# SamsungLabs/Metis

Hardware: NVIDIA H100
Metric: candidate plans evaluated/sec (higher is better)
Workload: dtype f64

## Files before the change

metis_b200/csrc/metis_eval.cuh:

```cuda
#pragma once

#include <stdint.h>
#include <string.h>
#include <math.h>

#include "../../include/metis_b200.h"

#if defined(__CUDACC__)
#define MB_HD __host__ __device__ __forceinline__
#define MB_HD_NOINLINE __host__ __device__ __noinline__
#else
#define MB_HD inline
#define MB_HD_NOINLINE inline
#endif

namespace metis {

constexpr int kH = 7;
constexpr double kMemCoef = 5.0;
constexpr uint8_t kDropped = 0xFF;

struct Tables {
    MetisProblem p;
    const int16_t *key_index;
// ... 45 lines not shown
    if (i < d.dpk) return (double)(i - d.ratio) / (double)p.num_layers;
    const double bw = bw_first[0] * 1048576.0;
    if (i < d.pp_hidden) {
        const int dp = 1 << (i - d.dpk);
        return (double)(2 * (dp - 1)) / ((double)dp * bw);
    }
    if (i < d.pp_vocab) return (double)((int64_t)(i - d.pp_hidden) * p.sequence_length * p.hidden_size) / bw;
    if (i >= d.dsub) return norm_lc[(i - d.dsub) / kH] / 7.0;
    if (i >= d.psub) {
        const int j = i - d.psub, r = j / kH;
        double acc = 0.0;
        for (int t = 0; t < r; ++t) acc += norm_lc[t];
        return r < p.norm_len ? acc + norm_lc[r] * ((double)(j - r * kH) / 7.0) : acc;
    }
    const int e = i - d.pp_vocab;
    const int mbs = e / p.num_tp, tpc = e - mbs * p.num_tp;
    return ((double)((int64_t)mbs * p.sequence_length * p.vocab_size) / (double)(1 << tpc)) / bw;
}

MB_HD void bind_derived(Tables &T, const double *base) {
    const DerivedLayout d = derived_layout(T.p);
    T.dlay = base + d.dlay;
    T.inv_exec = base + d.inv_exec;
    T.ratio = base + d.ratio;
    T.dpk = base + d.dpk;
    T.pp_hidden = base + d.pp_hidden;
    T.pp_vocab = base + d.pp_vocab;
    T.psub = base + d.psub;
    T.dsub = base + d.dsub;
}

struct PlanDesc {
    uint32_t ordinal;
    int ns;
    int S;
    int label;
    int batches;
    const uint8_t *row;
    uint64_t geo;
};

MB_HD uint64_t pack_geo(int64_t row_offset, int S, int label, int ns, int div) {
    return (uint64_t)(row_offset & 0xFFFFFFFFLL) | ((uint64_t)((S - 1) & 0xFF) << 32) | ((uint64_t)((label - 1) & 0xFF) << 40) |
           ((uint64_t)(ns & 0xFF) << 48) | ((uint64_t)(div & 0xFF) << 56);
}

enum BalancerPath {
    kPathVerifyFailed = 0,
    kPathSeqForward = 1,
    kPathIrregular = 2,
    kPathMiddle = 3,
    kPathFirstGe = 4,
    kPathTail = 5,
};

struct Serial {
    static constexpr bool kUniform = false;
    MB_HD void mark(int) const {}
    MB_HD void note(int) const {}
    MB_HD void converge() const {}
    MB_HD void rejoin(bool) {}
};
#if defined(__CUDACC__)
struct Lockstep : Serial {
    unsigned mask;
    __device__ Lockstep() : mask(0xFFFFFFFFu) {}
    __device__ void converge() const { __syncwarp(mask); }
    __device__ void rejoin(bool p) { mask = __ballot_sync(0xFFFFFFFFu, p); }
};
#endif
struct SerialUniform : Serial {
    static constexpr bool kUniform = true;
};

constexpr uint64_t kOnes = 0x0101010101010101ULL;

constexpr uint16_t kBroke = 0x8000;
constexpr uint16_t kTaken = 0x4000;
constexpr uint16_t kPos = 0x3FFF;

template <int MAXS, int MAXL>
struct Scratch {
    double perf[MAXS];
    double capa[MAXS];
    double mstate[MAXS];
    double extra[MAXS];
    uint16_t fe[MAXS];
    uint16_t first[MAXS], lastl[MAXS], cnt[MAXS];
    uint16_t part[MAXS + 1];
    uint16_t rs[MAXS + 1];
    uint8_t gcode[MAXS];
    uint8_t tpc[MAXS];
    uint8_t lstk[MAXS];
    uint8_t got[MAXS];
    uint64_t ownerw[MAXL / 8 + 1];
    uint64_t subw[MAXL];
    static_assert(MAXL >= MAXS, "after the vote, subw holds one double per stage (adjust_performance, get_cost)");
};

MB_HD double py_sum_range(const double *x, int a, int b) {
    if (a >= b) return 0.0;
    double f = 0.0 + x[a];
    double c = 0.0;
    for (int i = a + 1; i < b; ++i) {
        const double v = x[i];
        const double t = f + v;
        if (fabs(f) >= fabs(v)) c += (f - t) + v;
        else c += (v - t) + f;
        f = t;
    }
    if (c != 0.0 && isfinite(c)) f += c;
    return f;
}

MB_HD_NOINLINE double py_sum_range_compact(const double *x, int a, int b) {
    if (a >= b) return 0.0;
    double f = 0.0 + x[a];
    double c = 0.0;
#pragma unroll 1
    for (int i = a + 1; i < b; ++i) {
        const double v = x[i];
        const double t = f + v;
        if (fabs(f) >= fabs(v)) c += (f - t) + v;
        else c += (v - t) + f;
        f = t;
    }
    if (c != 0.0 && isfinite(c)) f += c;
    return f;
}

template <class X>
MB_HD double sum_range(const double *x, int a, int b) {
    if constexpr (X::kUniform) return py_sum_range_compact(x, a, b);
    else return py_sum_range(x, a, b);
}

MB_HD void fill_range_sums(const double *row, int L, int a, double *out) {
    const int n = L + 1;
    double f = 0.0 + row[a];
    double c = 0.0;
    out[(size_t)(a + 1) * n + a] = f;
#if defined(__CUDA_ARCH__)
#pragma unroll 1
#endif
    for (int i = a + 1; i < L; ++i) {
        const double v = row[i];
        const double t = f + v;
        if (fabs(f) >= fabs(v)) c += (f - t) + v;
        else c += (v - t) + f;
        f = t;
// ... 38 lines not shown
        ++n;
    }
    MB_HD double result() const {
        double r = f;
        if (c != 0.0 && isfinite(c)) r += c;
        return r;
    }
};

MB_HD double pow2_neg(int k) {
    const uint64_t bits = (uint64_t)(1023 - k) << 52;
    double d;
    memcpy(&d, &bits, sizeof(d));
    return d;
}

MB_HD int type_of_rank(const Tables &T, int ns, int rank) {
    const int nt = T.p.num_types;
    const int32_t *end = T.run_end + ns * nt;
    const uint8_t *typ = T.run_type + ns * nt;
#pragma unroll 1
    for (int k = 0; k < nt; ++k)
        if (rank < end[k]) return typ[k];
    return typ[nt - 1];
}

MB_HD int type_of_q10(const Tables &T, int ns, int idx) {
    const int nt = T.p.num_types;
    const int32_t *end = T.q10_end + ns * nt;
    const uint8_t *typ = T.run_type + ns * nt;
#pragma unroll 1
    for (int k = 0; k < nt; ++k)
        if (idx < end[k]) return typ[k];
    return typ[nt - 1];
}

MB_HD int key_of(const Tables &T, int type, int tpc, int bs) {
    if (tpc >= T.p.num_tp || bs < 1 || bs > T.p.num_bs) return -1;
    return T.key_index[(type * T.p.num_tp + tpc) * T.p.num_bs + (bs - 1)];
}

template <int MAXS, int MAXL>
MB_HD int fwd_start(const Scratch<MAXS, MAXL> &w, int s) {
    if (s == 0) return 0;
    const uint16_t e = w.fe[s - 1];
    return (e & kPos) + ((e & kBroke) ? 1 : 0);
}

template <int MAXS, int MAXL>
MB_HD bool fwd_nonempty(const Scratch<MAXS, MAXL> &w, int s) {
    return (int)(w.fe[s] & kPos) > fwd_start(w, s);
}

MB_HD void sub_store(uint64_t *subw, int j, int stage) {
    reinterpret_cast<uint8_t *>(subw)[(j / kH) * 8 + (j % kH)] = (uint8_t)stage;
}

MB_HD int popc64(uint64_t v) {
#if defined(__CUDA_ARCH__)
    return __popcll(v);
#else
    return __builtin_popcountll(v);
#endif
}
MB_HD int ctz64(uint64_t v) {
#if defined(__CUDA_ARCH__)
    return __ffsll((long long)v) - 1;
#else
    return __builtin_ctzll(v);
#endif
}
MB_HD int popc32(uint32_t v) {
#if defined(__CUDA_ARCH__)
    return __popc(v);
#else
    return __builtin_popcount(v);
#endif
}
MB_HD int ctz32(uint32_t v) {
#if defined(__CUDA_ARCH__)
    return __ffs((int)v) - 1;
#else
    return __builtin_ctz(v);
#endif
}
MB_HD int clz32(uint32_t v) {
#if defined(__CUDA_ARCH__)
    return __clz((int)v);
#else
    return __builtin_clz(v);
#endif
}
MB_HD int clz64(uint64_t v) {
#if defined(__CUDA_ARCH__)
    return __clzll((long long)v);
#else
    return __builtin_clzll(v);
#endif
}

MB_HD uint64_t swar_eq(uint64_t x, int c) {
    const uint64_t y = x ^ ((uint64_t)c * kOnes);
    const uint64_t lo7 = 0x7F7F7F7F7F7F7F7FULL;
    return ~((((y & lo7) + lo7) | y) | lo7);
}

MB_HD int swar_count(uint64_t x, int c) { return popc64(swar_eq(x, c) & 0x0080808080808080ULL); }

MB_HD int layer_owner(uint64_t v, bool plurality) {
    if (plurality) {
        int best = 0, own = (int)kDropped;
#pragma unroll 1
        for (int q = 0; q < kH; ++q) {
            const int cq = (int)((v >> (8 * q)) & 0xFF);
            const int n = swar_count(v, cq);
            if (n > best || (n == best && cq < own)) { best = n; own = cq; }
        }
        return own;
    }
    const int c3 = (int)((v >> 24) & 0xFF);
    if (swar_count(v, c3) * 2 > kH) return c3;
    const int c0 = (int)(v & 0xFF), c1 = (int)((v >> 8) & 0xFF), c2 = (int)((v >> 16) & 0xFF);
    if (swar_count(v, c0) * 2 > kH) return c0;
    if (c1 != c0 && swar_count(v, c1) * 2 > kH) return c1;
    if (c2 != c1 && c2 != c0 && swar_count(v, c2) * 2 > kH) return c2;
    return (int)kDropped;
}

template <int MAXS, int MAXL, class X>
MB_HD int balance_run(const Tables &T, int S, Scratch<MAXS, MAXL> &w, const X &x) {
    const int L = T.p.num_layers;
    if (T.p.norm_len < L) return METIS_FATAL_INDEX;
    const double *dlay = T.dlay;
    const double *lc = T.norm_lc;
    const int N = kH * L;
    const int lim = (N - 1 - kH) > 0 ? (N - 1 - kH) : 0;
    const int last = S - 1;
    int broken = METIS_FATAL_NONE;

#pragma unroll (X::kUniform ? 1 : 0)
    for (int s = 0; s < S; ++s) { w.capa[s] = w.perf[s]; w.got[s] = 0; w.cnt[s] = 0; }

    x.mark(10);
    int k = 0, sTop = -1;
    bool topSkip = false;
    if (S > 1) {
        int s = 0, j = 0;
        double c = w.capa[0];
#pragma unroll (X::kUniform ? 1 : 0)
        for (int r = 0; r + 1 < L; ++r) {
            const double d = dlay[r];
            const int nsub = (r == L - 2) ? kH - 1 : kH;
            const int s_in = s;
            uint64_t v = 0;
#pragma unroll
            for (int q = 0; q < kH; ++q) {
                if (q < nsub) {
                    if (s < last) {
                        if (c > d) {
                            c -= d;
                            v |= (uint64_t)(uint32_t)s << (8 * q);
                        } else {
                            w.capa[s] = c;
                            w.fe[s] = (uint16_t)(j | kBroke);
                            ++s;
                            c = w.capa[s];
                        }
                    }
                    ++j;
                }
            }
            if (s_in < last) w.subw[r] = v;
        }
        if (s < last) {
            x.note(kPathTail);
            w.capa[s] = c;
            w.fe[s] = (uint16_t)lim;
#pragma unroll (X::kUniform ? 1 : 0)
            for (int t = s + 1; t < last; ++t) w.fe[t] = (uint16_t)lim;
            k = lim;
            sTop = s;
        } else {
            k = (w.fe[last - 1] & kPos) + 1;
            sTop = last - 1;
            topSkip = true;
        }
    }

    x.mark(11);
    x.converge();
    int m;
    {
        double c = w.capa[last];
        const double dl = dlay[L - 1];
#pragma unroll (X::kUniform ? 1 : 0)
        for (int i = 0; i < kH; ++i) c -= dl;
        m = N - kH;
        int sp = S - 2;
#pragma unroll (X::kUniform ? 1 : 0)
        while (m > 0) {
            const int j = m - 1;
            bool un = (j >= k);
            if (!un) {
#pragma unroll (X::kUniform ? 1 : 0)
                while (sp >= 0 && (!(w.fe[sp] & kBroke) || (int)(w.fe[sp] & kPos) > j)) --sp;
                un = (sp >= 0 && (int)(w.fe[sp] & kPos) == j);
            }
            if (!un) break;
            const double d = dlay[j / kH];
            if (!(c > d)) break;
            c -= d;
            m = j;
            if (j < k) w.fe[sp] |= kTaken;
        }
        w.capa[last] = c;
    }

    x.mark(12);
    x.converge();
    {
        int start = 0;
#pragma unroll (X::kUniform ? 1 : 0)
        for (int s = 0; s < last; ++s) {
            const uint16_t e = w.fe[s];
            const int pos = e & kPos;
            const int next_start = pos + ((e & kBroke) ? 1 : 0);
            if ((e & (kBroke | kTaken)) != kBroke) { start = next_start; continue; }
            const int j = pos;
            int lo = 0;
            if (pos > start) {
                lo = s;
            } else {
                x.note(kPathIrregular);
#pragma unroll (X::kUniform ? 1 : 0)
                for (int u = s;; --u) {
                    if (u < s) {
                        const int t = w.lstk[u];
                        const bool above = (t == last) || (fwd_nonempty(w, t) && fwd_start(w, t) > j);
                        if (!above) { lo = t; break; }
                    }
                    if (fwd_nonempty(w, u)) { lo = u; break; }
                    if (u == 0) break;
                }
            }
            int hi = s + 1;
            if (hi < last && !((int)(w.fe[hi] & kPos) > next_start && !w.got[hi])) {
                ++hi;
#pragma unroll (X::kUniform ? 1 : 0)
                while (hi < last && (!fwd_nonempty(w, hi) || w.got[hi])) ++hi;
            }
            if (lo > hi) { broken = METIS_FATAL_SCRATCH; hi = lo; }
            int pick = lo;
            double best = w.capa[lo];
#pragma unroll (X::kUniform ? 1 : 0)
            for (int t = lo + 1; t <= hi; ++t)
                if (w.capa[t] > best) { best = w.capa[t]; pick = t; }
            w.capa[pick] -= dlay[j / kH];
            w.lstk[s] = (uint8_t)pick;
            w.got[pick] = 1;
            sub_store(w.subw, j, pick);
            start = next_start;
        }
    }
    x.converge();
    const int nblk = m - k;
    if (nblk > 0) x.note(kPathMiddle);
    {
        int below = -1;
#pragma unroll (X::kUniform ? 1 : 0)
        for (int t = 0; t < nblk; ++t) {
            const int j = k + t;
            int lo = 0;
            if (below >= 0) lo = below;
            else if (sTop >= 0) {
#pragma unroll (X::kUniform ? 1 : 0)
                for (int u = sTop;; --u) {
                    if (u < sTop || topSkip) {
                        const uint16_t eu = w.fe[u];
                        if ((eu & (kBroke | kTaken)) == kBroke) {
                            const int t2 = w.lstk[u];
                            if (t2 != last) { lo = t2; break; }
                        }
                    }
                    if (fwd_nonempty(w, u)) { lo = u; break; }
                    if (u == 0) break;
                }
            }
            int pick = lo;
            double best = w.capa[lo];
#pragma unroll (X::kUniform ? 1 : 0)
            for (int t2 = lo + 1; t2 <= last; ++t2)
                if (w.capa[t2] > best) { best = w.capa[t2]; pick = t2; }
            w.capa[pick] -= dlay[j / kH];
            if (pick != last) below = pick;
            sub_store(w.subw, j, pick);
        }
    }

    x.mark(13);
    x.converge();
    int run_own = (int)kDropped, run_first = 0, run_len = 0;
#pragma unroll (X::kUniform ? 1 : 0)
    for (int r = 0; r < L; ++r) {
        const int nlow = m - kH * r;
        int own;
        if (nlow <= 0) {
            own = last;
        } else {
            uint64_t v = w.subw[r];
            if (nlow < kH) {
                const uint64_t mask = (1ULL << (8 * nlow)) - 1ULL;
                v = (v & mask) | (((uint64_t)last * kOnes) & ~mask);
            }
            v |= 0xFF00000000000000ULL;
            own = layer_owner(v, (T.p.corrected & METIS_FIX_Q5) != 0);
        }
        reinterpret_cast<uint8_t *>(w.ownerw)[r] = (uint8_t)own;
        {
            if (own == run_own) ++run_len;
            else {
                if (run_own != (int)kDropped) {
                    if (w.cnt[run_own] == 0) w.first[run_own] = (uint16_t)run_first;
                    w.lastl[run_own] = (uint16_t)(r - 1);
                    w.cnt[run_own] = (uint16_t)(w.cnt[run_own] + run_len);
                }
                run_own = own; run_first = r; run_len = 1;
            }
        }
    }
    if (run_own != (int)kDropped) {
        if (w.cnt[run_own] == 0) w.first[run_own] = (uint16_t)run_first;
        w.lastl[run_own] = (uint16_t)(L - 1);
        w.cnt[run_own] = (uint16_t)(w.cnt[run_own] + run_len);
    }
    x.mark(14);
    x.converge();
    uint8_t *owner = reinterpret_cast<uint8_t *>(w.ownerw);
#pragma unroll (X::kUniform ? 1 : 0)
    for (int s = 0; s < S; ++s)
        w.capa[s] = w.cnt[s] ? w.perf[s] - range_sum<X>(T, kRangeNorm, 0, lc, w.first[s], (int)w.lastl[s] + 1) : w.perf[s];

    x.mark(15);
    x.converge();
#pragma unroll (X::kUniform ? 1 : 0)
    for (int n = 1; n <= 3; ++n) {
        int top = 0x7FFFFFFF;
        double maxc = -INFINITY;
#pragma unroll (X::kUniform ? 1 : 0)
        for (int t = 0; t < S; ++t)
            if (w.capa[t] > maxc) { maxc = w.capa[t]; top = t; }
        if (top == 0x7FFFFFFF) top = 0;
        int nb = -1;
        double val = INFINITY;
        if (top - 1 >= 0 && w.capa[top - 1] < val) { nb = top - 1; val = w.capa[top - 1]; }
        if (top + 1 < S && w.capa[top + 1] < val) { nb = top + 1; }
        if (nb < 0 || w.cnt[nb] <= 1) break;
        const int layer = (top > nb) ? w.lastl[nb] : w.first[nb];
        const double dl = lc[layer];
        const double ntop = w.capa[top] - dl;
        const double nnb = w.capa[nb] + dl;
        double newmax = -INFINITY;
#pragma unroll (X::kUniform ? 1 : 0)
        for (int t = 0; t < S; ++t) {
            const double v = (t == top) ? ntop : (t == nb) ? nnb : w.capa[t];
            if (v > newmax) newmax = v;
        }
        if (newmax > maxc) break;
        owner[layer] = (uint8_t)top;
        w.capa[top] = ntop;
        w.capa[nb] = nnb;
        if (top > nb) { int r = layer - 1; while (owner[r] != nb) --r; w.lastl[nb] = (uint16_t)r; }
        else          { int r = layer + 1; while (owner[r] != nb) ++r; w.first[nb] = (uint16_t)r; }
        if (w.cnt[top] == 0) { w.first[top] = (uint16_t)layer; w.lastl[top] = (uint16_t)layer; }
        else {
            if (layer < (int)w.first[top]) w.first[top] = (uint16_t)layer;
            if (layer > (int)w.lastl[top]) w.lastl[top] = (uint16_t)layer;
        }
        ++w.cnt[top];
        --w.cnt[nb];
    }

    x.mark(16);
    x.converge();
    w.part[0] = 0;
#pragma unroll (X::kUniform ? 1 : 0)
    for (int s = 0; s < S; ++s) w.part[s + 1] = (uint16_t)(w.part[s] + w.cnt[s]);
    return broken;
}

struct HSplit {
    int nruns;
    int type[METIS_MAX_TYPES];
    int n[METIS_MAX_TYPES];
    int base[METIS_MAX_TYPES];
    int plus[METIS_MAX_TYPES];
};

MB_HD_NOINLINE int partition_data(const Tables &T, int ns, int rank_lo, int count, int dp, int tpc, int bs,
                                  HSplit &out, uint32_t &aux, bool q10 = false) {
    const int gsz = count / dp;
    double perf[METIS_MAX_TYPES];
    PySum total;
    out.nruns = 0;
#pragma unroll 1
    for (int i = 0; i < dp; ++i) {
        const int t = q10 ? type_of_q10(T, ns, rank_lo + i * gsz) : type_of_rank(T, ns, rank_lo + i * gsz);
        if (out.nruns == 0 || out.type[out.nruns - 1] != t) {
            const int key = key_of(T, t, tpc, 1);
            if (key < 0) { aux = ((uint32_t)tpc << 16) | 1u; return METIS_FATAL_KEY_EXEC; }
            const double e = T.exec_full[key];
            if (e == 0.0) return METIS_FATAL_ZERODIV;
            out.type[out.nruns] = t;
            out.n[out.nruns] = 0;
            perf[out.nruns] = 1. / e;
            ++out.nruns;
        }
        ++out.n[out.nruns - 1];
        total.add(perf[out.nruns - 1]);
    }
    const double tot = total.result();
    double frac[METIS_MAX_TYPES];
    int assigned = 0;
#pragma unroll 1
    for (int r = 0; r < out.nruns; ++r) {
        const double v = (double)bs * (perf[r] / tot);
        const int b = (int)v;
        out.base[r] = b;
        out.plus[r] = 0;
        frac[r] = v - (double)b;
        assigned += b * out.n[r];
    }
    int rem = bs - assigned;
// ... 232 lines not shown
    MB_HD bool stage_time(int s, double &len) {
        const bool one_type = ONE || T.p.num_types == 1;
        const int g = w.gcode[s], tpc = w.tpc[s];
        const int a = one_type ? 0 : rank_start(s), b = a + (1 << g);
        const int la = w.part[s], lb = w.part[s + 1];
        const int ldp = g - tpc;
        const int ta = one_type ? 0 : type_of_rank(T, pd.ns, a);
        const int tb = one_type ? 0 : type_of_rank(T, pd.ns, b - 1);
        len = 0.0;
        if (ta != tb) return hetero_exec_cost(a, b, 1 << ldp, tpc, la, lb, len) != 0;
        const int key = key_of(T, ta, tpc, bs_total >> ldp);
        if (key < 0) return true;
        len = range_sum<X>(T, kRangeLc, key, T.lc + (size_t)key * T.p.lpad, la, lb);
        return false;
    }

    MB_HD void stage_terms(int s, int nstage, double &pp, double &dpc, double &upd) const {
        const int per = T.p.devices_per_node;
        const int Lm = T.p.num_layers;
        const bool ubw = T.p.uniform_bw != 0;
        const int g = w.gcode[s], tpc = w.tpc[s];
        const int la = w.part[s], lb = w.part[s + 1];
        const int ldp = g - tpc;
        const int mbs = bs_total >> ldp;
        const double inv_tp = pow2_neg(tpc);
        pp = 0.0;
        if (s < nstage - 1) {
            if (ubw) {
                pp = (lb == Lm - 1) ? T.pp_vocab[mbs * T.p.num_tp + tpc] : T.pp_hidden[mbs];
            } else {
                double act;
                if (lb == Lm - 1)
                    act = (double)((int64_t)mbs * T.p.sequence_length * T.p.vocab_size) * inv_tp;
                else
                    act = (double)((int64_t)mbs * T.p.sequence_length * T.p.hidden_size);
                pp = act / (bw_of_node_range(rank_start(s) / per, (rank_start(s + 2) - 1) / per) * 1048576.0);
            }
        }
        int ntr = lb - la;
        double params = 0.0;
        if (la == 0) { params += T.p.input_params * inv_tp; --ntr; }
        if (lb == Lm) { params += T.p.output_params * inv_tp; --ntr; }
        params += T.p.transformer_params * inv_tp * (double)ntr;
        if (ubw) dpc = T.dpk[ldp] * params;
        else {
            const int dp = 1 << ldp;
            dpc = (double)(2 * (dp - 1)) / ((double)dp * (dp_bandwidth(rank_start(s), dp, 1 << tpc) * 1048576.0)) * params;
        }
        upd = T.p.optimizer_time * inv_tp * T.ratio[lb - la];
    }


    MB_HD int compute_performance() {
#pragma unroll (X::kUniform ? 1 : 0)
        for (int s = 0; s < pd.S; ++s) {
            double p;
            const int rc = stage_performance(s, p);
            w.perf[s] = p;
            w.extra[s] = encode_error(rc, aux);
        }
        x.converge();
        PySum total;
#pragma unroll (X::kUniform ? 1 : 0)
        for (int s = 0; s < pd.S; ++s) {
            if (w.extra[s] != 0.0) return decode_error(w.extra[s], aux);
            total.add(w.perf[s]);
        }
        const double tot = total.result();
        if (tot == 0.0) return METIS_FATAL_ZERODIV;
#pragma unroll (X::kUniform ? 1 : 0)
        for (int s = 0; s < pd.S; ++s) w.perf[s] = w.perf[s] / tot;
        return 0;
    }

    MB_HD_NOINLINE int hetero_memory_demand(int s, int type0, double &demand) {
        const int la = w.part[s], lb = w.part[s + 1], tpc = w.tpc[s];
        HSplit hs;
        const int rc = partition_data(T, pd.ns, 0, T.p.q10_devices, dp_of(s), tpc, bs_total, hs, aux, true);
        if (rc) return rc;
#pragma unroll (X::kUniform ? 1 : 0)
        for (int r = 0; r < hs.nruns; ++r)
#pragma unroll (X::kUniform ? 1 : 0)
            for (int i = 0; i < hs.n[r]; ++i) {
                const int h = hs.base[r] + (i < hs.plus[r] ? 1 : 0);
#pragma unroll (X::kUniform ? 1 : 0)
                for (int bit = 30; bit >= 0; --bit) {
                    const int piece = 1 << bit;
                    if (!(h & piece)) continue;
                    const int key = key_of(T, type0, tpc, piece);
                    if (key < 0) { aux = ((uint32_t)tpc << 16) | (uint32_t)piece; return METIS_FATAL_KEY_MEMORY; }
                    demand += range_sum<X>(T, kRangeMem, key, T.mem + (size_t)key * T.p.lpad, la, lb) * kMemCoef;
                }
            }
        return 0;
    }

    MB_HD_NOINLINE int memory_demand_own_type(int s, double &demand) {
        const int la = w.part[s], lb = w.part[s + 1], tpc = w.tpc[s], g = w.gcode[s];
        const int a = rank_start(s), b = a + (1 << g);
        const int ta = type_of_rank(T, pd.ns, a), tb = type_of_rank(T, pd.ns, b - 1);
        if (ta == tb) {
            const int bs = bs_total >> (g - tpc);
            const int key = key_of(T, ta, tpc, bs);
            if (key < 0) { aux = ((uint32_t)tpc << 16) | (uint32_t)bs; return METIS_FATAL_KEY_MEMORY; }
            demand += range_sum<SerialUniform>(T, kRangeMem, key, T.mem + (size_t)key * T.p.lpad, la, lb) * kMemCoef;
            return 0;
        }
        HSplit hs;
        const int rc = partition_data(T, pd.ns, a, b - a, 1 << (g - tpc), tpc, bs_total, hs, aux);
        if (rc) return rc;
        double worst = 0.0;
#pragma unroll 1
        for (int r = 0; r < hs.nruns; ++r)
#pragma unroll 1
            for (int v = 0; v < 2; ++v) {
                const int cntv = v ? hs.plus[r] : hs.n[r] - hs.plus[r];
                const int h = hs.base[r] + v;
                if (cntv <= 0 || h == 0) continue;
                double need = 0.0;
#pragma unroll 1
                for (int bit = 30; bit >= 0; --bit) {
                    const int piece = 1 << bit;
                    if (!(h & piece)) continue;
                    const int key = key_of(T, hs.type[r], tpc, piece);
                    if (key < 0) { aux = ((uint32_t)tpc << 16) | (uint32_t)piece; return METIS_FATAL_KEY_MEMORY; }
                    need += range_sum<SerialUniform>(T, kRangeMem, key, T.mem + (size_t)key * T.p.lpad, la, lb) * kMemCoef;
                }
                if (need > worst) worst = need;
            }
        demand += worst;
        return 0;
    }

    MB_HD_NOINLINE int adjust_performance() {
        const int S = pd.S;
        double *ratio = reinterpret_cast<double *>(w.subw);
        double need = 0.;
        PySum avail_sum;
#pragma unroll (X::kUniform ? 1 : 0)
        for (int s = 0; s < S; ++s) {
            double av, adj, extra;
            stage_adjust(s, av, adj, extra);
            w.capa[s] = av;
            w.mstate[s] = adj;
            need += extra;
            avail_sum.add(av);
        }
        if (avail_sum.result() < need) return 1;
#pragma unroll (X::kUniform ? 1 : 0)
        for (int s = 0; s < S; ++s) w.extra[s] = 0.;
        int guard = 0;
#pragma unroll (X::kUniform ? 1 : 0)
        while (need > 0.01) {
            PySum tot;
#pragma unroll (X::kUniform ? 1 : 0)
            for (int s = 0; s < S; ++s) tot.add(w.capa[s] > 0.001 ? w.perf[s] : 0.0);
            const double tmp_total = tot.result();
#pragma unroll (X::kUniform ? 1 : 0)
            for (int s = 0; s < S; ++s)
                ratio[s] = w.capa[s] > 0.001 ? w.perf[s] / tmp_total : 0.0;
#pragma unroll (X::kUniform ? 1 : 0)
            for (int s = 0; s < S; ++s) {
                const double av = w.capa[s];
                const double want = need * ratio[s];
                const double give = want > av ? av : want;
                w.extra[s] += give;
                w.capa[s] -= give;
                need -= give;
            }
            if (++guard > 4096) return -METIS_FATAL_HANG;
        }
#pragma unroll (X::kUniform ? 1 : 0)
        for (int s = 0; s < S; ++s) w.perf[s] = w.extra[s] + w.mstate[s];
        return 0;
    }

    MB_HD int memory_phase(int attempt) {
        const int S = pd.S;
#pragma unroll (X::kUniform ? 1 : 0)
        for (int s = 0; s < S; ++s) {
            double md, state;
            const int rc = stage_memory(s, md, state);
            w.extra[s] = md;
            w.capa[s] = state;
            w.mstate[s] = encode_error(rc, aux);
            if (tap) { tap->demand[s] = md; tap->state[s] = state; }
        }
        x.converge();
        bool oom = false;
#pragma unroll (X::kUniform ? 1 : 0)
        for (int s = 0; s < S; ++s) {
            if (w.mstate[s] != 0.0) return -decode_error(w.mstate[s], aux);
            if (w.capa[s] < 0) oom = true;
        }
        if (!oom) {
#pragma unroll (X::kUniform ? 1 : 0)
            for (int s = 0; s < S; ++s) w.mstate[s] = w.capa[s];
            return 1;
        }
        if (attempt >= 3) return 0;
        x.mark(21);
        const int rc = adjust_performance();
        if (rc < 0) return rc;
        return rc == 1 ? 0 : 2;
    }

    template <class Sink>
    MB_HD_NOINLINE int partition_layer(Sink &sink) {
#pragma unroll (X::kUniform ? 1 : 0)
        for (int attempt = 1; attempt <= 3; ++attempt) {
            sink.balancer_run();
            const int rc = balance_run<MAXS, MAXL>(T, pd.S, w, x);
            if (rc) return -rc;
            const int r = memory_phase(attempt);
            if (r == 1) return attempt;
            if (r <= 0) return r;
        }
        return 0;
    }

    MB_HD double bw_of_node_range(int n0, int n1) const {
        const int per = T.p.devices_per_node;
        if (n0 == n1) return T.bw_first[type_of_q10(T, pd.ns, n0 * per)];
        double slow = INFINITY;
        const int nt = T.p.num_types;
        const int32_t *end = T.q10_end + pd.ns * nt;
        const uint8_t *typ = T.run_type + pd.ns * nt;
        int lo = 0;
#pragma unroll (X::kUniform ? 1 : 0)
        for (int k = 0; k < nt; ++k) {
            const int hi = end[k];
            if (hi > lo && n0 * per < hi && (n1 + 1) * per > lo) {
                const double v = T.bw_min[typ[k]];
                if (v < slow) slow = v;
            }
            lo = hi;
        }
        return slow;
    }

    MB_HD double dp_bandwidth(int a, int dp, int tp) const {
        const int per = T.p.devices_per_node;
        double slow = INFINITY;
#pragma unroll (X::kUniform ? 1 : 0)
        for (int d = 0; d < dp; ++d) {
            const int n0 = (a + d) / per;
            int nlast = n0;
            bool multi = false;
            double gmin = INFINITY;
            int tprev = -1;
#pragma unroll (X::kUniform ? 1 : 0)
            for (int i = 0; i < tp; ++i) {
                const int node = (a + d + i * dp) / per;
                if (node != nlast) { multi = true; nlast = node; }
                const int t = type_of_q10(T, pd.ns, node * per);
                if (t != tprev) { const double v = T.bw_min[t]; if (v < gmin) gmin = v; tprev = t; }
            }
// ... 7 lines not shown
        HSplit hs;
        uint32_t dummy;
        if (partition_data(T, pd.ns, a, b - a, dp, tpc, bs_total, hs, dummy)) return 1;
        len = -INFINITY;
#pragma unroll (X::kUniform ? 1 : 0)
        for (int r = 0; r < hs.nruns; ++r)
#pragma unroll (X::kUniform ? 1 : 0)
            for (int v = 0; v < 2; ++v) {
                const int cntv = v ? hs.plus[r] : hs.n[r] - hs.plus[r];
                const int h = hs.base[r] + v;
                if (cntv <= 0 || h == 0) continue;
                double acc = 0.;
#pragma unroll (X::kUniform ? 1 : 0)
                for (int bit = 30; bit >= 0; --bit) {
                    const int piece = 1 << bit;
                    if (!(h & piece)) continue;
                    if (piece > T.p.max_bs) return 1;
                    const int key = key_of(T, hs.type[r], tpc, piece);
                    if (key < 0) return 1;
                    acc += range_sum<X>(T, kRangeLc, key, T.lc + (size_t)key * T.p.lpad, la, lb);
                }
                if (acc > len) len = acc;
            }
        return 0;
    }

    MB_HD int fb_sync_cost(int a, int b, int tpc, int mbs, double &out) const {
        const int nt = T.p.num_types;
        const int32_t *end = T.run_end + pd.ns * nt;
        const uint8_t *typ = T.run_type + pd.ns * nt;
        double mx = -INFINITY;
        int lo = 0;
#pragma unroll (X::kUniform ? 1 : 0)
        for (int k = 0; k < nt; ++k) {
            const int hi = end[k];
            if ((a > lo ? a : lo) < (b < hi ? b : hi)) {
                const int key = key_of(T, typ[k], tpc, mbs);
                if (key < 0) return 1;
                const double v = T.fb_sync[key];
                if (v == 0.0) return 1;
                if (v > mx) mx = v;
            }
            lo = hi;
        }
        out = mx;
        return 0;
    }

    MB_HD int get_cost(double &cost_out) {
        const bool one_type = ONE || T.p.num_types == 1;
        const int nstage = pd.label < pd.S ? pd.label : pd.S;
        if (T.p.q10_devices < T.p.total_devices && rank_start(nstage) > T.p.q10_devices) return 1;
        bool bad = false;
#pragma unroll (X::kUniform ? 1 : 0)
        for (int s = 0; s < nstage; ++s) {
            double len;
            if (stage_time(s, len)) bad = true;
            w.capa[s] = len;
        }
        if (bad) return 1;
        double *ppterm = reinterpret_cast<double *>(w.subw);
        double max_len = -INFINITY, max_upd = -INFINITY, max_dp = -INFINITY;
#pragma unroll (X::kUniform ? 1 : 0)
        for (int s = 0; s < nstage; ++s) {
            double dpc, upd;
            stage_terms(s, nstage, ppterm[s], dpc, upd);
            if (w.capa[s] > max_len) max_len = w.capa[s];
            if (dpc > max_dp) max_dp = dpc;
            if (upd > max_upd) max_upd = upd;
        }
        PySum lens_sum;
        double pp_cost = 0., fb_sync = 0.;
#pragma unroll (X::kUniform ? 1 : 0)
        for (int s = 0; s < nstage; ++s) {
            lens_sum.add(w.capa[s]);
            if (s < nstage - 1) pp_cost += ppterm[s];
        }
        {
            const int s = nstage - 1;
            const int a = one_type ? 0 : rank_start(s), b = a + group(s);
            double v;
            if (fb_sync_cost(a, b, w.tpc[s], bs_total >> (w.gcode[s] - w.tpc[s]), v)) return 1;
            fb_sync = v * (double)pd.batches;
        }
        const double exec = ((double)(pd.batches - 1) * max_len) + lens_sum.result();
        const double bg = T.p.batch_generator * (double)pd.batches;
        cost_out = exec + fb_sync + max_upd + max_dp + pp_cost + bg;
        if (tap) { tap->cost[0] = exec; tap->cost[1] = fb_sync; tap->cost[2] = max_upd; tap->cost[3] = max_dp; tap->cost[4] = pp_cost; }
        return 0;
    }

    template <class Sink>
    MB_HD_NOINLINE void run(const PlanDesc &plan, Sink &sink, int only_step = -1) {
        const int ok = begin(plan);
        if (ok < 0) { sink.fatal(plan.ordinal, METIS_FATAL_SCRATCH, 0); return; }
        if (ok == 0) return;
        bool started = false, have_state = false;
        int nrep = 0, step = 0;
#pragma unroll (X::kUniform ? 1 : 0)
        for (;;) {
            if (nrep == 1) return;
            int attempt = 0;
#pragma unroll (X::kUniform ? 1 : 0)
            for (;;) {
                if (!started) started = true;
                else if (!next_strategy(have_state)) return;
                if (!valid()) continue;
                sink.partition_call();
                int rc = compute_performance();
                if (rc) { sink.fatal(pd.ordinal, rc, aux); return; }
                attempt = partition_layer(sink);
                if (attempt < 0) { sink.fatal(pd.ordinal, -attempt, aux); return; }
                have_state = attempt > 0;
                if (attempt > 0) break;
            }
            nrep = attempt;
            double cost;
            if (get_cost(cost) == 0) sink.emit(pd, step, nrep, cost, w.tpc, w.part);
            else sink.keyerror();
            if (only_step >= 0 && step == only_step) return;
            ++step;
        }
    }
};

template <int MAXS, int MAXL, bool ONE, class X = Serial, class Sink>
MB_HD bool first_task(const Tables &T, Scratch<MAXS, MAXL> &w, Sink &sink, bool has, const PlanDesc &plan, int &chain_hint,
                      int &resume) {
    PlanEvaluator<MAXS, MAXL, X, ONE> ev(T, w);
// ... 116 lines not shown
```

metis_b200/csrc/metis_search.cu:

```cuda
#include <cuda_runtime.h>
#include <cooperative_groups.h>
#include <stdint.h>
#include <stdio.h>
#include <stdlib.h>
#include <string.h>

#include "metis_eval.cuh"
#include "metis_coop.cuh"
#include "metis_warp.cuh"
#include "metis_trace.cuh"
#include "metis_rows.cuh"

namespace cg = cooperative_groups;

namespace metis {

#ifndef METIS_THREADS
#define METIS_THREADS 256
#endif
#ifndef METIS_MIN_BLOCKS
#define METIS_MIN_BLOCKS 3
#endif
#ifndef METIS_MIN_BLOCKS_BIG
#define METIS_MIN_BLOCKS_BIG METIS_MIN_BLOCKS
// ... 171 lines not shown
    } else {
        lo = find_block(sp, ordinal);
    }
    const MetisPlanBlock b = sp.blocks[lo];
    const int64_t rel = ordinal - b.first_ordinal;
    const int64_t row = rel / sp.num_div;
    const int div = (int)(rel - row * sp.num_div);
    pd.ordinal = (uint32_t)ordinal;
    pd.ns = b.ns_idx;
    pd.S = b.num_stage;
    pd.label = b.label_stage;
    pd.batches = __ldg(&sp.batches[div]);
    const int64_t off = b.rows_offset + row * b.num_stage;
    pd.row = sp.rows + off;
    pd.geo = pack_geo(off, b.num_stage, b.label_stage, b.ns_idx, div);
    return true;
}

__device__ __forceinline__ void decode_task(const MetisPlanSpace &sp, uint64_t hdr, uint64_t geo, PlanDesc &pd) {
    pd.ordinal = (uint32_t)hdr;
    pd.geo = geo;
    pd.row = sp.rows + (geo & 0xFFFFFFFFULL);
    pd.S = (int)((geo >> 32) & 0xFF) + 1;
    pd.label = (int)((geo >> 40) & 0xFF) + 1;
    pd.ns = (int)((geo >> 48) & 0xFF);
    pd.batches = __ldg(&sp.batches[(geo >> 56) & 0xFF]);
}

__device__ __forceinline__ bool rec_less(double c0, uint32_t o0, uint32_t s0, double c1, uint32_t o1, uint32_t s1) {
    if (c0 < c1) return true;
    if (c0 > c1) return false;
    if (o0 != o1) return o0 < o1;
    return s0 < s1;
}

struct DeviceOut {
    MetisRecord *records;
    long long capacity;
    uint8_t *detail;
    int detail_stride;
    unsigned long long *counters;
    MetisRecord *block_best;
};

struct DeviceSink {
    const DeviceOut &o;
    unsigned int n_part, n_run, n_key;
    double best_cost;
    uint32_t best_ord, best_step, best_meta;
    bool leader;
    __device__ DeviceSink(const DeviceOut &out)
        : o(out), n_part(0), n_run(0), n_key(0), best_cost(INFINITY), best_ord(0xFFFFFFFFu), best_step(0xFFFFu),
          best_meta(0), leader(true) {}
    __device__ void phase(int) {}
    __device__ void partition_call() { n_part += leader ? 1u : 0u; }
    __device__ void balancer_run() { n_run += leader ? 1u : 0u; }
    __device__ void keyerror() { n_key += leader ? 1u : 0u; }
    __device__ void fatal(uint32_t ordinal, int code, uint32_t aux) {
        if (!leader) return;
        const unsigned long long key = ((unsigned long long)ordinal << 32) | ((unsigned long long)(code & 0xFF) << 24) |
                                       (unsigned long long)(((aux >> 16) & 0xFF) << 16) | (aux & 0xFFFF);
        atomicMin(&o.counters[4], key);
    }
    __device__ void emit(const PlanDesc &pd, int step, int nrep, double cost, const uint8_t *tpc, const uint16_t *part) {
        if (!leader) return;
        const unsigned long long slot = atomicAdd(&o.counters[0], 1ULL);
        if ((long long)slot < o.capacity) {
            MetisRecord r;
            r.cost = cost; r.ordinal = pd.ordinal; r.step = (uint16_t)step;
            r.num_repartition = (uint8_t)nrep; r.num_stage = (uint8_t)pd.S;
            o.records[slot] = r;
            if (o.detail) {
                uint8_t *d = o.detail + (size_t)slot * o.detail_stride;
                for (int s = 0; s < pd.S; ++s) { d[s] = (uint8_t)(pd.row[s] - tpc[s]); d[pd.S + s] = tpc[s]; }
                for (int s = 0; s <= pd.S; ++s) d[2 * pd.S + s] = (uint8_t)part[s];
            }
        }
        if (rec_less(cost, pd.ordinal, (uint32_t)step, best_cost, best_ord, best_step)) {
            best_cost = cost; best_ord = pd.ordinal; best_step = (uint32_t)step;
            best_meta = ((uint32_t)nrep << 8) | (uint32_t)pd.S;
        }
    }
};

__device__ __forceinline__ void finish_block(const DeviceSink &sink, const DeviceOut &out, int slot) {
    __shared__ double s_cost[32];
    __shared__ uint32_t s_ord[32], s_step[32], s_meta[32];
    const unsigned full = 0xFFFFFFFFu;
    const unsigned np = __reduce_add_sync(full, sink.n_part);
    const unsigned nr = __reduce_add_sync(full, sink.n_run);
    const unsigned nk = __reduce_add_sync(full, sink.n_key);
    const int lane = threadIdx.x & 31, warp = threadIdx.x >> 5;
    if (lane == 0) {
        if (np) atomicAdd(&out.counters[1], (unsigned long long)np);
        if (nr) atomicAdd(&out.counters[2], (unsigned long long)nr);
        if (nk) atomicAdd(&out.counters[3], (unsigned long long)nk);
    }
    double c = sink.best_cost;
    uint32_t o = sink.best_ord, st = sink.best_step, mt = sink.best_meta;
    for (int d = 16; d > 0; d >>= 1) {
        const double c2 = __shfl_xor_sync(full, c, d);
        const uint32_t o2 = __shfl_xor_sync(full, o, d), s2 = __shfl_xor_sync(full, st, d),
                       m2 = __shfl_xor_sync(full, mt, d);
        if (rec_less(c2, o2, s2, c, o, st)) { c = c2; o = o2; st = s2; mt = m2; }
    }
    if (lane == 0) { s_cost[warp] = c; s_ord[warp] = o; s_step[warp] = st; s_meta[warp] = mt; }
    __syncthreads();
// ... 374 lines not shown
    if (lane == 0) {
        cw.init(local, s_pool[wid]);
        for (uint32_t skip = 0; skip < rec.first_row; ++skip) cw.advance();
    }
    uint8_t *dst = rows + rec.row_offset;
    for (uint32_t r = 0;;) {
        __syncwarp();
        int at = 0;
        for (int h = cw.head; h >= 0; h = cw.nxt[h]) {
            const int len = cw.len[h], off = cw.off[h];
            for (int b = lane; b < len; b += 32) dst[at + b] = cw.codes[off + b];
            at += len;
        }
        __syncwarp();
        if (++r >= rec.num_rows) break;
        int more = 0;
        if (lane == 0) more = cw.advance() ? 1 : 0;
        if (!__shfl_sync(full, more, 0)) break;
        dst += stages;
    }
}

__global__ void divide_by_seven_kernel(const double *lc, int n, double *out) {
    const int i = blockIdx.x * blockDim.x + threadIdx.x;
    if (i < n) out[i] = lc[i] / 7.0;
}

static int check_problem(const MetisProblem *p) {
    if (!p) return arg_fail("problem is NULL");
    if (p->num_types < 1 || p->num_types > METIS_MAX_TYPES) return arg_fail("num_types out of range");
    if (p->num_layers < 1 || p->num_layers > METIS_MAX_LAYERS || p->num_layers > 255)
        return arg_fail("num_layers out of range (1 .. 255)");
    if (p->lpad < p->num_layers) return arg_fail("lpad < num_layers");
    if (p->num_keys < 1 || p->num_tp < 1 || p->num_bs < 1 || p->norm_len < 1) return arg_fail("empty profile tables");
    if (p->devices_per_node < 1 || p->total_devices < 1 || p->q10_devices < 1) return arg_fail("empty cluster");
    return METIS_OK;
}

}

using namespace metis;

extern "C" {

const char *metis_last_error(void) { return g_err; }
int metis_abi_version(void) { return METIS_ABI_VERSION; }
#ifdef METIS_PROFILE_PHASES
int metis_debug_marks(long long *out32, int reset) {
    long long zero[64] = {0};
    if (out32) cudaMemcpyFromSymbol(out32, g_mark_acc, sizeof(zero));
    if (reset) cudaMemcpyToSymbol(g_mark_acc, zero, sizeof(zero));
    return 0;
}
#endif
void metis_set_profile_events(void *before_kernel, void *after_kernel) {
    g_ev_before = static_cast<cudaEvent_t>(before_kernel);
    g_ev_after = static_cast<cudaEvent_t>(after_kernel);
}

static int64_t shard_plan_slots(int64_t num_plans, const MetisShard *sh) {
    const int64_t tile = sh->tile, world = sh->world;
    const int64_t rounds = (num_plans + tile * world - 1) / (tile * world);
    return rounds * tile;
}

constexpr int64_t kFixedWs = 16384;
constexpr int64_t kMaxBlocks = 4096;

static int env_int(const char *name, int lo, int hi, int dflt) {
    const char *e = getenv(name);
    if (!e || !*e) return dflt;
    char *end = nullptr;
    const long v = strtol(e, &end, 10);
    if (end == e || *end != '\0' || v < lo || v > hi) return dflt;
    return (int)v;
}

static int64_t save_slots(int64_t cap) {
    const int forced = env_int("METIS_SAVE_SLOTS", 1, 1 << 20, 0);
    if (forced) return forced;
    return cap / 4 < 131072 ? (cap / 4 > 0 ? cap / 4 : 1) : 131072;
}

int64_t metis_het_workspace_bytes(const MetisProblem *problem, int64_t num_plans, int32_t max_stage) {
    if (check_problem(problem)) return METIS_E_ARG;
    if (num_plans < 0) return METIS_E_ARG;
    const BlobLayout lay = make_layout(*problem);
    const int64_t cap = (num_plans + 127) & ~(int64_t)127;
    const int64_t stages = max_stage < 1 ? 1 : (max_stage > METIS_MAX_STAGES ? METIS_MAX_STAGES : max_stage);
    return 256 + kFixedWs + (int64_t)lay.rsum + (int64_t)align16(lay.rsum_bytes) + kMaxBlocks * (int64_t)sizeof(MetisRecord) +
           2 * cap * (int64_t)sizeof(uint4) + cap * 4 + save_slots(cap) * stages * 8 + 1024;
}

struct Workspace {
    MetisSearchSummary *summary;
    unsigned long long *counters;
    unsigned int *ctl;
    uint8_t *blob;
    MetisRecord *block_best;
    uint8_t *lists;
};

static Workspace carve(void *ws, const BlobLayout &lay) {
    uint8_t *b = static_cast<uint8_t *>(ws);
    uintptr_t a = (reinterpret_cast<uintptr_t>(b) + 127) & ~(uintptr_t)127;
    b = reinterpret_cast<uint8_t *>(a);
// ... 256 lines not shown
```

Measured before the change: 183.0 million.

## Reconstruct layer votes from stage boundaries instead of storing per-sublayer owners

The balancer no longer writes the owner of every sublayer into scratch during the forward and backward sweeps. The layer vote now rebuilds each sublayer's stage from the forward-end markers, the backward picks and a compact middle-block array. Other loops are fused: the capacity copy is folded into the sweep, the top-stage search is carried between iterations instead of rescanned, and the error-encoding passes in compute_performance, memory_phase, adjust_performance and get_cost are merged into single loops with early break. The aim is less scratch (local or shared memory) traffic, at the cost of a more complex vote loop with a nested while. A profiling-only bulk timing hook is also added behind a macro.

```diff
diff --git a/metis_b200/csrc/metis_eval.cuh b/metis_b200/csrc/metis_eval.cuh
--- a/metis_b200/csrc/metis_eval.cuh
+++ b/metis_b200/csrc/metis_eval.cuh
@@ -121,6 +121,7 @@
     kPathMiddle = 3,
     kPathFirstGe = 4,
     kPathTail = 5,
+    kPathVoteEnds = 6,
 };
 
 struct Serial {
@@ -130,12 +131,33 @@
     MB_HD void converge() const {}
     MB_HD void rejoin(bool) {}
 };
+#if defined(__CUDACC__) && defined(METIS_PROFILE_PHASES)
+constexpr int kBulkBatches = 31;
+__device__ long long g_bulk_acc[32];
+__shared__ long long s_bulk_t[32];
+__shared__ int s_bulk_cur[32];
+__device__ __forceinline__ void bulk_mark(unsigned group, int id) {
+    __syncwarp(group);
+    if ((int)(threadIdx.x & 31) == __ffs((int)group) - 1) {
+        const int wi = threadIdx.x >> 5;
+        const long long now = clock64();
+        if (id == 1) atomicAdd((unsigned long long *)&g_bulk_acc[kBulkBatches], 1ULL);
+        else atomicAdd((unsigned long long *)&g_bulk_acc[s_bulk_cur[wi] & 31], (unsigned long long)(now - s_bulk_t[wi]));
+        s_bulk_cur[wi] = id;
+        s_bulk_t[wi] = now;
+    }
+    __syncwarp(group);
+}
+#endif
 #if defined(__CUDACC__)
 struct Lockstep : Serial {
     unsigned mask;
     __device__ Lockstep() : mask(0xFFFFFFFFu) {}
     __device__ void converge() const { __syncwarp(mask); }
     __device__ void rejoin(bool p) { mask = __ballot_sync(0xFFFFFFFFu, p); }
+#if defined(METIS_PROFILE_PHASES)
+    __device__ void mark(int id) const { bulk_mark(__activemask(), id); }
+#endif
 };
 #endif
 struct SerialUniform : Serial {
@@ -164,7 +186,7 @@
     uint8_t got[MAXS];
     uint64_t ownerw[MAXL / 8 + 1];
     uint64_t subw[MAXL];
-    static_assert(MAXL >= MAXS, "after the vote, subw holds one double per stage (adjust_performance, get_cost)");
+    static_assert(MAXL >= MAXS, "after the vote, subw holds one double per stage (CoopEvaluator's adjust and cost)");
 };
 
 MB_HD double py_sum_range(const double *x, int a, int b) {
@@ -309,10 +331,6 @@
     return (int)(w.fe[s] & kPos) > fwd_start(w, s);
 }
 
-MB_HD void sub_store(uint64_t *subw, int j, int stage) {
-    reinterpret_cast<uint8_t *>(subw)[(j / kH) * 8 + (j % kH)] = (uint8_t)stage;
-}
-
 MB_HD int popc64(uint64_t v) {
 #if defined(__CUDA_ARCH__)
     return __popcll(v);
@@ -396,45 +414,41 @@
     int broken = METIS_FATAL_NONE;
 
 #pragma unroll (X::kUniform ? 1 : 0)
-    for (int s = 0; s < S; ++s) { w.capa[s] = w.perf[s]; w.got[s] = 0; w.cnt[s] = 0; }
+    for (int s = 0; s < S; ++s) { w.got[s] = 0; w.cnt[s] = 0; }
 
     x.mark(10);
     int k = 0, sTop = -1;
     bool topSkip = false;
     if (S > 1) {
         int s = 0, j = 0;
-        double c = w.capa[0];
+        double c = w.perf[0];
 #pragma unroll (X::kUniform ? 1 : 0)
         for (int r = 0; r + 1 < L; ++r) {
             const double d = dlay[r];
             const int nsub = (r == L - 2) ? kH - 1 : kH;
-            const int s_in = s;
-            uint64_t v = 0;
 #pragma unroll
             for (int q = 0; q < kH; ++q) {
                 if (q < nsub) {
                     if (s < last) {
                         if (c > d) {
                             c -= d;
-                            v |= (uint64_t)(uint32_t)s << (8 * q);
                         } else {
                             w.capa[s] = c;
                             w.fe[s] = (uint16_t)(j | kBroke);
                             ++s;
-                            c = w.capa[s];
+                            c = w.perf[s];
                         }
                     }
                     ++j;
                 }
             }
-            if (s_in < last) w.subw[r] = v;
         }
         if (s < last) {
             x.note(kPathTail);
             w.capa[s] = c;
             w.fe[s] = (uint16_t)lim;
 #pragma unroll (X::kUniform ? 1 : 0)
-            for (int t = s + 1; t < last; ++t) w.fe[t] = (uint16_t)lim;
+            for (int t = s + 1; t < last; ++t) { w.capa[t] = w.perf[t]; w.fe[t] = (uint16_t)lim; }
             k = lim;
             sTop = s;
         } else {
@@ -448,7 +462,7 @@
     x.converge();
     int m;
     {
-        double c = w.capa[last];
+        double c = w.perf[last];
         const double dl = dlay[L - 1];
 #pragma unroll (X::kUniform ? 1 : 0)
         for (int i = 0; i < kH; ++i) c -= dl;
@@ -515,13 +529,13 @@
             w.capa[pick] -= dlay[j / kH];
             w.lstk[s] = (uint8_t)pick;
             w.got[pick] = 1;
-            sub_store(w.subw, j, pick);
             start = next_start;
         }
     }
     x.converge();
     const int nblk = m - k;
     if (nblk > 0) x.note(kPathMiddle);
+    uint8_t *mid = reinterpret_cast<uint8_t *>(w.subw);
     {
         int below = -1;
 #pragma unroll (X::kUniform ? 1 : 0)
@@ -550,27 +564,38 @@
                 if (w.capa[t2] > best) { best = w.capa[t2]; pick = t2; }
             w.capa[pick] -= dlay[j / kH];
             if (pick != last) below = pick;
-            sub_store(w.subw, j, pick);
+            mid[t] = (uint8_t)pick;
         }
     }
 
     x.mark(13);
     x.converge();
+    if (k > 0) x.note(kPathVoteEnds);
+    int t = 0, nxt = 0;
+    uint16_t e = 0;
+    if (k > 0) { e = w.fe[0]; nxt = (int)(e & kPos) + ((e & kBroke) ? 1 : 0); }
+    const bool plurality = (T.p.corrected & METIS_FIX_Q5) != 0;
     int run_own = (int)kDropped, run_first = 0, run_len = 0;
 #pragma unroll (X::kUniform ? 1 : 0)
     for (int r = 0; r < L; ++r) {
-        const int nlow = m - kH * r;
-        int own;
-        if (nlow <= 0) {
-            own = last;
-        } else {
-            uint64_t v = w.subw[r];
-            if (nlow < kH) {
-                const uint64_t mask = (1ULL << (8 * nlow)) - 1ULL;
-                v = (v & mask) | (((uint64_t)last * kOnes) & ~mask);
-            }
-            v |= 0xFF00000000000000ULL;
-            own = layer_owner(v, (T.p.corrected & METIS_FIX_Q5) != 0);
+        int own = last;
+        if (kH * r < m) {
+            uint64_t v = 0xFF00000000000000ULL;
+#pragma unroll
+            for (int q = 0; q < kH; ++q) {
+                const int j = kH * r + q;
+                int st = last;
+                if (j < k) {
+#pragma unroll 1
+                    while (nxt <= j) { ++t; e = w.fe[t]; nxt = (int)(e & kPos) + ((e & kBroke) ? 1 : 0); }
+                    st = t;
+                    if (nxt - 1 == j && (e & kBroke)) st = (e & kTaken) ? last : (int)w.lstk[t];
+                } else if (j < m) {
+                    st = mid[j - k];
+                }
+                v |= (uint64_t)(uint32_t)st << (8 * q);
+            }
+            own = layer_owner(v, plurality);
         }
         reinterpret_cast<uint8_t *>(w.ownerw)[r] = (uint8_t)own;
         {
@@ -593,19 +618,19 @@
     x.mark(14);
     x.converge();
     uint8_t *owner = reinterpret_cast<uint8_t *>(w.ownerw);
-#pragma unroll (X::kUniform ? 1 : 0)
-    for (int s = 0; s < S; ++s)
-        w.capa[s] = w.cnt[s] ? w.perf[s] - range_sum<X>(T, kRangeNorm, 0, lc, w.first[s], (int)w.lastl[s] + 1) : w.perf[s];
+    int top = 0x7FFFFFFF;
+    double maxc = -INFINITY;
+#pragma unroll (X::kUniform ? 1 : 0)
+    for (int s = 0; s < S; ++s) {
+        const double c = w.cnt[s] ? w.perf[s] - range_sum<X>(T, kRangeNorm, 0, lc, w.first[s], (int)w.lastl[s] + 1) : w.perf[s];
+        w.capa[s] = c;
+        if (c > maxc) { maxc = c; top = s; }
+    }
 
     x.mark(15);
     x.converge();
 #pragma unroll (X::kUniform ? 1 : 0)
     for (int n = 1; n <= 3; ++n) {
-        int top = 0x7FFFFFFF;
-        double maxc = -INFINITY;
-#pragma unroll (X::kUniform ? 1 : 0)
-        for (int t = 0; t < S; ++t)
-            if (w.capa[t] > maxc) { maxc = w.capa[t]; top = t; }
         if (top == 0x7FFFFFFF) top = 0;
         int nb = -1;
         double val = INFINITY;
@@ -617,10 +642,11 @@
         const double ntop = w.capa[top] - dl;
         const double nnb = w.capa[nb] + dl;
         double newmax = -INFINITY;
+        int newtop = 0x7FFFFFFF;
 #pragma unroll (X::kUniform ? 1 : 0)
         for (int t = 0; t < S; ++t) {
             const double v = (t == top) ? ntop : (t == nb) ? nnb : w.capa[t];
-            if (v > newmax) newmax = v;
+            if (v > newmax) { newmax = v; newtop = t; }
         }
         if (newmax > maxc) break;
         owner[layer] = (uint8_t)top;
@@ -635,6 +661,8 @@
         }
         ++w.cnt[top];
         --w.cnt[nb];
+        maxc = newmax;
+        top = newtop;
     }
 
     x.mark(16);
@@ -973,20 +1001,18 @@
 
 
     MB_HD int compute_performance() {
+        PySum total;
+        int rc = 0;
 #pragma unroll (X::kUniform ? 1 : 0)
         for (int s = 0; s < pd.S; ++s) {
             double p;
-            const int rc = stage_performance(s, p);
+            rc = stage_performance(s, p);
+            if (rc) break;
             w.perf[s] = p;
-            w.extra[s] = encode_error(rc, aux);
+            total.add(p);
         }
         x.converge();
-        PySum total;
-#pragma unroll (X::kUniform ? 1 : 0)
-        for (int s = 0; s < pd.S; ++s) {
-            if (w.extra[s] != 0.0) return decode_error(w.extra[s], aux);
-            total.add(w.perf[s]);
-        }
+        if (rc) return rc;
         const double tot = total.result();
         if (tot == 0.0) return METIS_FATAL_ZERODIV;
 #pragma unroll (X::kUniform ? 1 : 0)
@@ -1055,7 +1081,6 @@
 
     MB_HD_NOINLINE int adjust_performance() {
         const int S = pd.S;
-        double *ratio = reinterpret_cast<double *>(w.subw);
         double need = 0.;
         PySum avail_sum;
 #pragma unroll (X::kUniform ? 1 : 0)
@@ -1064,12 +1089,11 @@
             stage_adjust(s, av, adj, extra);
             w.capa[s] = av;
             w.mstate[s] = adj;
+            w.extra[s] = 0.;
             need += extra;
             avail_sum.add(av);
         }
         if (avail_sum.result() < need) return 1;
-#pragma unroll (X::kUniform ? 1 : 0)
-        for (int s = 0; s < S; ++s) w.extra[s] = 0.;
         int guard = 0;
 #pragma unroll (X::kUniform ? 1 : 0)
         while (need > 0.01) {
@@ -1078,12 +1102,10 @@
             for (int s = 0; s < S; ++s) tot.add(w.capa[s] > 0.001 ? w.perf[s] : 0.0);
             const double tmp_total = tot.result();
 #pragma unroll (X::kUniform ? 1 : 0)
-            for (int s = 0; s < S; ++s)
-                ratio[s] = w.capa[s] > 0.001 ? w.perf[s] / tmp_total : 0.0;
-#pragma unroll (X::kUniform ? 1 : 0)
             for (int s = 0; s < S; ++s) {
                 const double av = w.capa[s];
-                const double want = need * ratio[s];
+                const double ratio = av > 0.001 ? w.perf[s] / tmp_total : 0.0;
+                const double want = need * ratio;
                 const double give = want > av ? av : want;
                 w.extra[s] += give;
                 w.capa[s] -= give;
@@ -1098,32 +1120,26 @@
 
     MB_HD int memory_phase(int attempt) {
         const int S = pd.S;
+        bool oom = false;
+        int rc = 0;
 #pragma unroll (X::kUniform ? 1 : 0)
         for (int s = 0; s < S; ++s) {
             double md, state;
-            const int rc = stage_memory(s, md, state);
+            rc = stage_memory(s, md, state);
+            if (rc) break;
             w.extra[s] = md;
-            w.capa[s] = state;
-            w.mstate[s] = encode_error(rc, aux);
+            w.mstate[s] = state;
+            if (state < 0) oom = true;
             if (tap) { tap->demand[s] = md; tap->state[s] = state; }
         }
         x.converge();
-        bool oom = false;
-#pragma unroll (X::kUniform ? 1 : 0)
-        for (int s = 0; s < S; ++s) {
-            if (w.mstate[s] != 0.0) return -decode_error(w.mstate[s], aux);
-            if (w.capa[s] < 0) oom = true;
-        }
-        if (!oom) {
-#pragma unroll (X::kUniform ? 1 : 0)
-            for (int s = 0; s < S; ++s) w.mstate[s] = w.capa[s];
-            return 1;
-        }
+        if (rc) return -rc;
+        if (!oom) return 1;
         if (attempt >= 3) return 0;
         x.mark(21);
-        const int rc = adjust_performance();
-        if (rc < 0) return rc;
-        return rc == 1 ? 0 : 2;
+        const int adj = adjust_performance();
+        if (adj < 0) return adj;
+        return adj == 1 ? 0 : 2;
     }
 
     template <class Sink>
@@ -1237,29 +1253,25 @@
         const int nstage = pd.label < pd.S ? pd.label : pd.S;
         if (T.p.q10_devices < T.p.total_devices && rank_start(nstage) > T.p.q10_devices) return 1;
         bool bad = false;
+        PySum lens_sum;
+        double max_len = -INFINITY;
 #pragma unroll (X::kUniform ? 1 : 0)
         for (int s = 0; s < nstage; ++s) {
             double len;
             if (stage_time(s, len)) bad = true;
-            w.capa[s] = len;
+            lens_sum.add(len);
+            if (len > max_len) max_len = len;
         }
         if (bad) return 1;
-        double *ppterm = reinterpret_cast<double *>(w.subw);
-        double max_len = -INFINITY, max_upd = -INFINITY, max_dp = -INFINITY;
+        double max_upd = -INFINITY, max_dp = -INFINITY;
+        double pp_cost = 0., fb_sync = 0.;
 #pragma unroll (X::kUniform ? 1 : 0)
         for (int s = 0; s < nstage; ++s) {
-            double dpc, upd;
-            stage_terms(s, nstage, ppterm[s], dpc, upd);
-            if (w.capa[s] > max_len) max_len = w.capa[s];
+            double pp, dpc, upd;
+            stage_terms(s, nstage, pp, dpc, upd);
+            if (s < nstage - 1) pp_cost += pp;
             if (dpc > max_dp) max_dp = dpc;
             if (upd > max_upd) max_upd = upd;
-        }
-        PySum lens_sum;
-        double pp_cost = 0., fb_sync = 0.;
-#pragma unroll (X::kUniform ? 1 : 0)
-        for (int s = 0; s < nstage; ++s) {
-            lens_sum.add(w.capa[s]);
-            if (s < nstage - 1) pp_cost += ppterm[s];
         }
         {
             const int s = nstage - 1;
diff --git a/metis_b200/csrc/metis_search.cu b/metis_b200/csrc/metis_search.cu
--- a/metis_b200/csrc/metis_search.cu
+++ b/metis_b200/csrc/metis_search.cu
@@ -247,7 +247,11 @@
     __device__ DeviceSink(const DeviceOut &out)
         : o(out), n_part(0), n_run(0), n_key(0), best_cost(INFINITY), best_ord(0xFFFFFFFFu), best_step(0xFFFFu),
           best_meta(0), leader(true) {}
+#ifdef METIS_PROFILE_PHASES
+    __device__ void phase(int id) { bulk_mark(0xFFFFFFFFu, id); }
+#else
     __device__ void phase(int) {}
+#endif
     __device__ void partition_call() { n_part += leader ? 1u : 0u; }
     __device__ void balancer_run() { n_run += leader ? 1u : 0u; }
     __device__ void keyerror() { n_key += leader ? 1u : 0u; }
@@ -728,6 +732,12 @@
     if (reset) cudaMemcpyToSymbol(g_mark_acc, zero, sizeof(zero));
     return 0;
 }
+int metis_debug_bulk_marks(long long *out32, int reset) {
+    long long zero[32] = {0};
+    if (out32) cudaMemcpyFromSymbol(out32, g_bulk_acc, sizeof(zero));
+    if (reset) cudaMemcpyToSymbol(g_bulk_acc, zero, sizeof(zero));
+    return 0;
+}
 #endif
 void metis_set_profile_events(void *before_kernel, void *after_kernel) {
     g_ev_before = static_cast<cudaEvent_t>(before_kernel);
```

After: 202.3 million, median of 6. 1.11x the previous value.
